# sparsemat/sprs

Measured on NVIDIA H100. Metric: csr_spmv_f64_gflops, higher is better.
Workload: dtype f64

## Files before the change

### include/sprs_b200.h

```cpp
#ifndef SPRS_B200_H
#define SPRS_B200_H

#include <stddef.h>
#include <stdint.h>

#ifdef __cplusplus
extern "C" {
#endif

typedef struct sprs_b200_ctx sprs_b200_ctx;
typedef struct sprs_b200_csmat sprs_b200_csmat;
typedef struct sprs_b200_spgemm sprs_b200_spgemm;

enum { SPRS_B200_CSR = 0, SPRS_B200_CSC = 1 };

enum {
    SPRS_B200_OK = 0,
    SPRS_B200_ERR_DIMENSION = 1,
    SPRS_B200_ERR_STORAGE = 2,
    SPRS_B200_ERR_CUDA = 3,
    SPRS_B200_ERR_NCCL = 4,
    SPRS_B200_ERR_INDEX_RANGE = 5,
    SPRS_B200_ERR_ARGUMENT = 6,
    SPRS_B200_ERR_STRUCTURE = 7,
// ... 186 lines not shown
enum { SPRS_B200_TRI_LOWER = 0, SPRS_B200_TRI_UPPER = 1 };
enum {
    SPRS_B200_SINGULAR_IS_ZERO = 0,
    SPRS_B200_SINGULAR_NUMERIC = 1,
    SPRS_B200_SINGULAR_STRUCTURAL = 2
};
int sprs_b200_trisolve_plan(sprs_b200_ctx* ctx, const sprs_b200_csmat* mat, int tri,
                            sprs_b200_trisolve** out);
int sprs_b200_trisolve_singular(const sprs_b200_trisolve* plan, uint64_t* index, int* reason);
int sprs_b200_trisolve_solve(sprs_b200_trisolve* plan, double* rhs, uint64_t len);
int sprs_b200_trisolve_solve_dev(sprs_b200_trisolve* plan, double* d_rhs, void* stream);
int sprs_b200_trisolve_free(sprs_b200_trisolve* plan);

typedef struct sprs_b200_ldl sprs_b200_ldl;
int sprs_b200_is_symmetric(sprs_b200_ctx* ctx, const sprs_b200_csmat* mat, int* out);
int sprs_b200_diag_solve(sprs_b200_ctx* ctx, const double* diag, double* x, uint64_t len);
int sprs_b200_ldl_symbolic(sprs_b200_ctx* ctx, const sprs_b200_csmat* mat, const uint32_t* perm,
                           int check_symmetry, sprs_b200_ldl** out);
uint64_t sprs_b200_ldl_nnz(const sprs_b200_ldl* ldl);
int sprs_b200_ldl_factor(const sprs_b200_ldl* sym, const sprs_b200_csmat* mat,
                         sprs_b200_ldl** out);
int sprs_b200_ldl_update(sprs_b200_ldl* num, const sprs_b200_csmat* mat);
int sprs_b200_ldl_singular(const sprs_b200_ldl* num, uint64_t* index);
int sprs_b200_ldl_solve(sprs_b200_ldl* num, const double* b, double* x, uint64_t len);
int sprs_b200_ldl_solve_dev(sprs_b200_ldl* num, const double* d_b, double* d_x, void* stream);
int sprs_b200_ldl_get_l(const sprs_b200_ldl* num, uint32_t* colptr, uint32_t* indices,
                        double* data);
int sprs_b200_ldl_get_d(const sprs_b200_ldl* num, double* d, uint64_t len);
int sprs_b200_ldl_free(sprs_b200_ldl* ldl);

int sprs_b200_diag_gather_ceiling(sprs_b200_ctx* ctx, const sprs_b200_csmat* mat,
                                  const double* d_x, int iters, double* ms_per_pass,
                                  uint64_t* nnz_covered);

int sprs_b200_gen_rmat_keys(sprs_b200_ctx* ctx, uint64_t seed, int scale, uint64_t n_rows,
                            uint64_t n_cols, double a, double b, double c, uint64_t first,
                            uint64_t count, uint64_t* d_keys, void* stream);
int sprs_b200_gen_uniform_keys(sprs_b200_ctx* ctx, uint64_t seed, uint64_t n_rows,
                               uint64_t n_cols, uint64_t first, uint64_t count,
                               uint64_t* d_keys, void* stream);
int sprs_b200_gen_normal_from_keys(sprs_b200_ctx* ctx, uint64_t seed, const uint64_t* d_keys,
                                   uint64_t count, double* d_out, void* stream);
int sprs_b200_gen_split_keys(sprs_b200_ctx* ctx, const uint64_t* d_keys, uint64_t count,
                             uint32_t* d_rows, uint32_t* d_cols, void* stream);
int sprs_b200_gen_hash_keys(sprs_b200_ctx* ctx, uint64_t seed, const uint64_t* d_keys,
                            uint64_t count, uint64_t* d_out, void* stream);

#ifdef __cplusplus
}
#endif
#endif
```

### rust/sprs-b200-sys/src/lib.rs

```rust
#![allow(non_camel_case_types)]
use std::os::raw::{c_char, c_double, c_int, c_void};

#[repr(C)] pub struct sprs_b200_ctx { _private: [u8; 0] }
#[repr(C)] pub struct sprs_b200_csmat { _private: [u8; 0] }
#[repr(C)] pub struct sprs_b200_spgemm { _private: [u8; 0] }
#[repr(C)] pub struct sprs_b200_comm { _private: [u8; 0] }
#[repr(C)] pub struct sprs_b200_symm { _private: [u8; 0] }
#[repr(C)] pub struct sprs_b200_bicgstab { _private: [u8; 0] }
#[repr(C)] pub struct sprs_b200_trisolve { _private: [u8; 0] }
#[repr(C)] pub struct sprs_b200_ldl { _private: [u8; 0] }

pub const SPRS_B200_CSR: c_int = 0;
pub const SPRS_B200_CSC: c_int = 1;
pub const SPRS_B200_BINOP_ADD: c_int = 0;
pub const SPRS_B200_BINOP_SUB: c_int = 1;
pub const SPRS_B200_BINOP_MUL: c_int = 2;
pub const SPRS_B200_OK: c_int = 0;
pub const SPRS_B200_ERR_DIMENSION: c_int = 1;
pub const SPRS_B200_ERR_STORAGE: c_int = 2;
pub const SPRS_B200_ERR_CUDA: c_int = 3;
pub const SPRS_B200_ERR_NCCL: c_int = 4;
pub const SPRS_B200_ERR_INDEX_RANGE: c_int = 5;
pub const SPRS_B200_ERR_ARGUMENT: c_int = 6;
pub const SPRS_B200_ERR_STRUCTURE: c_int = 7;
// ... 178 lines not shown
    pub fn sprs_b200_comm_unique_id(id: *mut c_char) -> c_int;
    pub fn sprs_b200_comm_init_rank(
        ctx: *mut sprs_b200_ctx, id: *const c_char, rank: c_int, world: c_int,
        out: *mut *mut sprs_b200_comm) -> c_int;
    pub fn sprs_b200_comm_free(comm: *mut sprs_b200_comm) -> c_int;
    pub fn sprs_b200_comm_rank(comm: *const sprs_b200_comm) -> c_int;
    pub fn sprs_b200_comm_world(comm: *const sprs_b200_comm) -> c_int;
    pub fn sprs_b200_comm_multicast_supported(comm: *const sprs_b200_comm) -> c_int;
    pub fn sprs_b200_comm_allgather_host(
        comm: *mut sprs_b200_comm, mine: *const c_void, bytes: u64, all: *mut c_void) -> c_int;
    pub fn sprs_b200_comm_barrier_host(comm: *mut sprs_b200_comm) -> c_int;
    pub fn sprs_b200_comm_barrier_dev(comm: *mut sprs_b200_comm, stream: *mut c_void) -> c_int;
    pub fn sprs_b200_comm_check(comm: *mut sprs_b200_comm, stream: *mut c_void) -> c_int;
    pub fn sprs_b200_symm_alloc(
        comm: *mut sprs_b200_comm, bytes: u64, want_multicast: c_int,
        out: *mut *mut sprs_b200_symm) -> c_int;
    pub fn sprs_b200_symm_free(buf: *mut sprs_b200_symm) -> c_int;
    pub fn sprs_b200_symm_ptr(buf: *const sprs_b200_symm, rank: c_int) -> *mut c_void;
    pub fn sprs_b200_symm_multicast_ptr(buf: *const sprs_b200_symm) -> *mut c_void;
    pub fn sprs_b200_symm_bytes(buf: *const sprs_b200_symm) -> u64;
    pub fn sprs_b200_partition_rows(
        indptr: *const c_void, indptr_bytes: c_int, rows: u64, nparts: c_int, row_cost: c_double,
        bounds: *mut u64) -> c_int;
    pub fn sprs_b200_spmv_rowpart(
        comm: *mut sprs_b200_comm, mat: *const sprs_b200_csmat, d_x: *const c_double,
        y: *mut sprs_b200_symm, row_offset: u64, exchange: c_int, stream: *mut c_void) -> c_int;
    pub fn sprs_b200_mul_mat_vec_rowpart(
        comm: *mut sprs_b200_comm, mat: *const sprs_b200_csmat, x: *mut sprs_b200_symm,
        x_slice: *const c_double, col_offset: u64, col_count: u64, y_slice: *mut c_double,
        y_len: u64) -> c_int;
    pub fn sprs_b200_diag_gather_ceiling(
        ctx: *mut sprs_b200_ctx, mat: *const sprs_b200_csmat, d_x: *const c_double, iters: c_int,
        ms_per_pass: *mut c_double, nnz_covered: *mut u64) -> c_int;
    pub fn sprs_b200_spmv_chunked_push_dev(
        ctx: *mut sprs_b200_ctx, mat: *const sprs_b200_csmat, d_x: *const c_double,
        row_offset: u64, n_targets: c_int, d_y_bufs: *const *mut c_double, accumulate: c_int,
        n_chunks: c_int, stream: *mut c_void) -> c_int;
    pub fn sprs_b200_spgemm_numeric_dev(
        ctx: *mut sprs_b200_ctx, plan: *mut sprs_b200_spgemm, c: *mut *mut sprs_b200_csmat) -> c_int;
    pub fn sprs_b200_spgemm_nprod(plan: *const sprs_b200_spgemm) -> u64;
    pub fn sprs_b200_bicgstab_new_dev(
        ctx: *mut sprs_b200_ctx, mat: *const sprs_b200_csmat, d_x0: *const c_double,
        d_b: *const c_double, n: u64, out: *mut *mut sprs_b200_bicgstab) -> c_int;
    pub fn sprs_b200_bicgstab_get_dev(
        s: *const sprs_b200_bicgstab, which: c_int, d_out: *mut *const c_double) -> c_int;
    pub fn sprs_b200_gen_rmat_keys(
        ctx: *mut sprs_b200_ctx, seed: u64, scale: c_int, n_rows: u64, n_cols: u64, a: c_double,
        b: c_double, c: c_double, first: u64, count: u64, d_keys: *mut u64, stream: *mut c_void) -> c_int;
    pub fn sprs_b200_gen_uniform_keys(
        ctx: *mut sprs_b200_ctx, seed: u64, n_rows: u64, n_cols: u64, first: u64, count: u64,
        d_keys: *mut u64, stream: *mut c_void) -> c_int;
    pub fn sprs_b200_gen_normal_from_keys(
        ctx: *mut sprs_b200_ctx, seed: u64, d_keys: *const u64, count: u64, d_out: *mut c_double,
        stream: *mut c_void) -> c_int;
    pub fn sprs_b200_gen_split_keys(
        ctx: *mut sprs_b200_ctx, d_keys: *const u64, count: u64, d_rows: *mut u32,
        d_cols: *mut u32, stream: *mut c_void) -> c_int;
    pub fn sprs_b200_gen_hash_keys(
        ctx: *mut sprs_b200_ctx, seed: u64, d_keys: *const u64, count: u64, d_out: *mut u64,
        stream: *mut c_void) -> c_int;
}
```

### sprs_b200/_lib.py

```python
import ctypes as C
import os

_HERE = os.path.dirname(os.path.abspath(__file__))
LIB_PATH = os.path.join(_HERE, "libsprs_b200.so")

OK, ERR_DIMENSION, ERR_STORAGE, ERR_CUDA, ERR_NCCL, ERR_INDEX_RANGE, ERR_ARGUMENT, \
    ERR_STRUCTURE, ERR_UNSUPPORTED = range(9)
CSR, CSC = 0, 1
BINOP_ADD, BINOP_SUB, BINOP_MUL = 0, 1, 2
ERR_SINGULAR = 10
ERR_NOT_SYMMETRIC = 11
TRI_LOWER, TRI_UPPER = 0, 1
SINGULAR_IS_ZERO, SINGULAR_NUMERIC, SINGULAR_STRUCTURAL = 0, 1, 2

_vp, _u64, _i64, _int, _dp = C.c_void_p, C.c_uint64, C.c_int64, C.c_int, C.c_void_p
_dense_sig = [_vp, _vp, _dp, _u64, _u64, _i64, _i64, _dp, _u64, _u64, _i64, _i64]

MATVEC_FN = C.CFUNCTYPE(C.c_int, C.c_void_p, C.c_void_p, C.c_void_p, C.c_void_p)

PROTOTYPES = {
    "sprs_b200_version": (_int, []),
    "sprs_b200_ctx_create": (_int, [_int, C.POINTER(_vp)]),
    "sprs_b200_ctx_destroy": (_int, [_vp]),
    "sprs_b200_last_error": (C.c_char_p, [_vp]),
# ... 68 lines not shown
    "sprs_b200_spgemm_free": (_int, [_vp]),
    "sprs_b200_bicgstab_new": (_int, [_vp, _vp, _dp, _dp, _u64, C.POINTER(_vp)]),
    "sprs_b200_bicgstab_new_dev": (_int, [_vp, _vp, _dp, _dp, _u64, C.POINTER(_vp)]),
    "sprs_b200_bicgstab_new_op": (_int, [_vp, _u64, MATVEC_FN, _vp, _dp, _dp, _int,
                                         C.POINTER(_vp)]),
    "sprs_b200_bicgstab_free": (_int, [_vp]),
    "sprs_b200_bicgstab_step": (_int, [_vp, C.POINTER(C.c_double)]),
    "sprs_b200_bicgstab_soft_restart": (_int, [_vp]),
    "sprs_b200_bicgstab_hard_restart": (_int, [_vp]),
    "sprs_b200_bicgstab_solve": (_int, [_vp, C.c_double, _u64, C.POINTER(_int)]),
    "sprs_b200_bicgstab_set_restart_threshold": (_int, [_vp, C.c_double]),
    "sprs_b200_bicgstab_stats": (_int, [_vp, C.POINTER(_u64), C.POINTER(C.c_double)]),
    "sprs_b200_bicgstab_get": (_int, [_vp, _int, _dp, _u64]),
    "sprs_b200_bicgstab_get_dev": (_int, [_vp, _int, C.POINTER(_vp)]),
    "sprs_b200_trisolve_plan": (_int, [_vp, _vp, _int, C.POINTER(_vp)]),
    "sprs_b200_trisolve_singular": (_int, [_vp, C.POINTER(_u64), C.POINTER(_int)]),
    "sprs_b200_trisolve_solve": (_int, [_vp, _dp, _u64]),
    "sprs_b200_trisolve_solve_dev": (_int, [_vp, _dp, _vp]),
    "sprs_b200_trisolve_free": (_int, [_vp]),
    "sprs_b200_diag_solve": (_int, [_vp, _dp, _dp, _u64]),
    "sprs_b200_is_symmetric": (_int, [_vp, _vp, C.POINTER(_int)]),
    "sprs_b200_ldl_symbolic": (_int, [_vp, _vp, _vp, _int, C.POINTER(_vp)]),
    "sprs_b200_ldl_nnz": (_u64, [_vp]),
    "sprs_b200_ldl_factor": (_int, [_vp, _vp, C.POINTER(_vp)]),
    "sprs_b200_ldl_update": (_int, [_vp, _vp]),
    "sprs_b200_ldl_singular": (_int, [_vp, C.POINTER(_u64)]),
    "sprs_b200_ldl_solve": (_int, [_vp, _dp, _dp, _u64]),
    "sprs_b200_ldl_solve_dev": (_int, [_vp, _dp, _dp, _vp]),
    "sprs_b200_ldl_get_l": (_int, [_vp, _vp, _vp, _dp]),
    "sprs_b200_ldl_get_d": (_int, [_vp, _dp, _u64]),
    "sprs_b200_ldl_free": (_int, [_vp]),
    "sprs_b200_diag_gather_ceiling": (_int, [_vp, _vp, _dp, _int, C.POINTER(C.c_double),
                                             C.POINTER(_u64)]),
    "sprs_b200_gen_rmat_keys": (_int, [_vp, _u64, _int, _u64, _u64, C.c_double, C.c_double,
                                       C.c_double, _u64, _u64, _vp, _vp]),
    "sprs_b200_gen_uniform_keys": (_int, [_vp, _u64, _u64, _u64, _u64, _u64, _vp, _vp]),
    "sprs_b200_gen_normal_from_keys": (_int, [_vp, _u64, _vp, _u64, _vp, _vp]),
    "sprs_b200_gen_split_keys": (_int, [_vp, _vp, _u64, _vp, _vp, _vp]),
    "sprs_b200_gen_hash_keys": (_int, [_vp, _u64, _vp, _u64, _vp, _vp]),
}

_NOT_EMULATED = ("sprs_b200_comm_", "sprs_b200_symm_", "sprs_b200_partition_rows",
                 "sprs_b200_spmv_rowpart", "sprs_b200_mul_mat_vec_rowpart", "sprs_b200_diag_",
                 "sprs_b200_csmat_binop", "sprs_b200_csmat_scale",
                 "sprs_b200_trisolve_",
                 "sprs_b200_ldl_", "sprs_b200_is_symmetric", "sprs_b200_diag_solve")
_lib = None


def load():
    global _lib
    if _lib is not None:
        return _lib
    if not os.path.exists(LIB_PATH):
        raise ImportError(
            "libsprs_b200.so is not built (%s): run `python -c 'import __graft_entry__ as g; "
            "g.build()'` or `make -C sprs_b200/csrc`.  sprs_b200 has no CPU fallback." % LIB_PATH)
    lib = C.CDLL(LIB_PATH)
    emulated = os.path.basename(LIB_PATH).startswith("libsprs_b200_emu")
    for name, (res, args) in PROTOTYPES.items():
        if emulated and name.startswith(_NOT_EMULATED) and not hasattr(lib, name):
            continue
        fn = getattr(lib, name)
        fn.restype = res
        fn.argtypes = args
    _lib = lib
# ... 2 lines not shown
```

### sprs_b200/csrc/api.cu

```cuda

#include <algorithm>
#include <mutex>
#include <vector>

#include <cstdlib>

#include "common.cuh"
#include "ptx.cuh"

namespace {

__global__ void make_policies_kernel(uint64_t* out) {
    out[0] = policy_evict_first();
    out[1] = policy_evict_last();
}

thread_local std::string g_create_error;

template <typename Src, typename Dst>
__global__ void convert_rebase_kernel(const Src* __restrict__ in, Dst* __restrict__ out,
                                      uint64_t n, uint64_t base) {
    const uint64_t i = blockIdx.x * (uint64_t)blockDim.x + threadIdx.x;
    if (i < n) out[i] = (Dst)((uint64_t)in[i] - base);
}
// ... 353 lines not shown
    m->d_indptr = const_cast<uint32_t*>(d_indptr);
    m->d_indices = const_cast<uint32_t*>(d_indices);
    m->d_data = const_cast<double*>(d_data);
    m->owns = false;
    int st = spmv_prepare(ctx, m, ctx->stream);
    if (st == SPRS_B200_OK && cudaStreamSynchronize(ctx->stream) != cudaSuccess) {
        sprs_b200_set_error(ctx, "from_device: partition kernel failed");
        st = SPRS_B200_ERR_CUDA;
    }
    if (st != SPRS_B200_OK) {
        sprs_b200_csmat_free(m);
        return st;
    }
    *out = m;
    return SPRS_B200_OK;
}

int sprs_b200_csmat_free(sprs_b200_csmat* m) {
    if (!m) return SPRS_B200_OK;
    if (m->ctx) cudaSetDevice(m->ctx->device);
    if (m->owns && m->pooled && m->ctx) {
        cudaDeviceSynchronize();
        if (m->d_indptr) cudaFreeAsync(m->d_indptr, m->ctx->stream);
        if (m->d_indices) cudaFreeAsync(m->d_indices, m->ctx->stream);
        if (m->d_data) cudaFreeAsync(m->d_data, m->ctx->stream);
    } else if (m->owns) {
        if (m->d_indptr) cudaFree(m->d_indptr);
        if (m->d_indices) cudaFree(m->d_indices);
        if (m->d_data) cudaFree(m->d_data);
    }
    if (m->d_tile_row) cudaFree(m->d_tile_row);
    if (m->d_tile_k) cudaFree(m->d_tile_k);
    if (m->d_carry) cudaFree(m->d_carry);
    if (m->d_hot_col) cudaFree(m->d_hot_col);
    if (m->d_hot_idx) cudaFree(m->d_hot_idx);
    if (m->csr_cache) sprs_b200_csmat_free(m->csr_cache);
    delete m;
    return SPRS_B200_OK;
}

static int csr_of(sprs_b200_ctx* ctx, const sprs_b200_csmat* m, const sprs_b200_csmat** out) {
    if (m->storage == SPRS_B200_CSR) {
        *out = m;
        return SPRS_B200_OK;
    }
    if (!m->csr_cache) {
        sprs_b200_csmat* t = nullptr;
        SPRS_TRY(sprs_b200_csmat_to_other_storage(ctx, m, &t));
        m->csr_cache = t;
    }
    *out = m->csr_cache;
    return SPRS_B200_OK;
}

int sprs_b200_csmat_storage(const sprs_b200_csmat* m) { return m ? m->storage : -1; }
uint64_t sprs_b200_csmat_rows(const sprs_b200_csmat* m) { return m ? m->rows : 0; }
uint64_t sprs_b200_csmat_cols(const sprs_b200_csmat* m) { return m ? m->cols : 0; }
uint64_t sprs_b200_csmat_nnz(const sprs_b200_csmat* m) { return m ? m->nnz : 0; }

int sprs_b200_csmat_download(sprs_b200_ctx* ctx, const sprs_b200_csmat* m, void* indptr,
                             int indptr_bytes, void* indices, int index_bytes, double* data) {
    if (!ctx || !m || !indptr) return SPRS_B200_ERR_ARGUMENT;
    if ((indptr_bytes != 4 && indptr_bytes != 8) || (index_bytes != 4 && index_bytes != 8))
        SPRS_FAIL(ctx, SPRS_B200_ERR_ARGUMENT, "bad index width");
    if (indptr_bytes == 4 && m->nnz > 0xffffffffull)
        SPRS_FAIL(ctx, SPRS_B200_ERR_INDEX_RANGE, "Index type is not large enough for nnz");
// ... 370 lines not shown
```

### sprs_b200/csrc/common.cuh

```cuda
#pragma once
#include <cuda_runtime.h>

#include <cstdint>
#include <cstdio>
#include <cstring>
#include <string>
#include <vector>

#include "../../include/sprs_b200.h"

constexpr int SPRS_E2E_MAX_CHUNKS = 8;
constexpr int SPRS_E2E_DEFAULT_CHUNKS = 8;

struct sprs_b200_ctx {
    int device = 0;
    int sm_count = 132;
    size_t l2_bytes = 0;
    cudaStream_t stream = nullptr;
    std::string last_error;
    uint64_t launches = 0;
    uint64_t pol_evict_first = 0, pol_evict_last = 0;
    void* h_stage = nullptr;
    size_t h_stage_bytes = 0;
    void* d_scratch[4] = {nullptr, nullptr, nullptr, nullptr};
    size_t d_scratch_bytes[4] = {0, 0, 0, 0};
    cudaStream_t side_stream = nullptr;
    cudaEvent_t ev_fork = nullptr, ev_join = nullptr;
    cudaStream_t copy_stream = nullptr;
    cudaEvent_t ev_chunk[SPRS_E2E_MAX_CHUNKS] = {};
    cudaEvent_t ev_copied = nullptr;
};

struct sprs_b200_csmat {
    sprs_b200_ctx* ctx = nullptr;
    int storage = SPRS_B200_CSR;
    uint64_t rows = 0, cols = 0, nnz = 0;
    uint64_t outer = 0, inner = 0;
    int indptr_bytes = 4;
    void* d_indptr = nullptr;
    uint32_t* d_indices = nullptr;
    double* d_data = nullptr;
    bool owns = true;
    bool pooled = false;
    uint32_t* d_tile_row = nullptr;
    void* d_tile_k = nullptr;
    double* d_carry = nullptr;
    uint64_t n_tiles = 0;
    uint32_t* d_hot_col = nullptr;
    uint32_t* d_hot_idx = nullptr;
    uint32_t n_hot = 0;
    mutable sprs_b200_csmat* csr_cache = nullptr;
    mutable std::vector<uint64_t> e2e_tiles, e2e_rows;
    mutable std::vector<uint64_t> push_tiles, push_rows;
};

#define SPRS_FAIL(ctx, code, ...)                                  \
    do {                                                           \
        char _buf[512];                                            \
        snprintf(_buf, sizeof(_buf), __VA_ARGS__);                 \
        sprs_b200_set_error((ctx), _buf);                          \
        return (code);                                             \
    } while (0)

#define SPRS_CUDA(ctx, expr)                                                              \
    do {                                                                                  \
        cudaError_t _e = (expr);                                                          \
        if (_e != cudaSuccess)                                                            \
            SPRS_FAIL((ctx), SPRS_B200_ERR_CUDA, "%s failed: %s (%s:%d)", #expr,          \
                      cudaGetErrorString(_e), __FILE__, __LINE__);                        \
    } while (0)

#define SPRS_TRY(expr)                      \
    do {                                    \
        int _s = (expr);                    \
        if (_s != SPRS_B200_OK) return _s;  \
    } while (0)

void sprs_b200_set_error(const sprs_b200_ctx* ctx, const char* msg);

// ... 84 lines not shown
```

### sprs_b200/csrc/diag.cu

```cuda
#include "common.cuh"
#include "ptx.cuh"

namespace {

constexpr int DIAG_EPL = 8, DIAG_NWARPS = 8, DIAG_CTAS = 2;

__global__ void __launch_bounds__(DIAG_NWARPS * 32, DIAG_CTAS)
    gather_ceiling_kernel(const uint32_t* __restrict__ idx, const double* __restrict__ val,
                          const double* __restrict__ x, double* __restrict__ out,
                          uint64_t n_tiles) {
    constexpr int WT = DIAG_EPL * 32;
    const int lane = threadIdx.x & 31, warp = threadIdx.x >> 5;
    const uint64_t gw = (uint64_t)blockIdx.x * DIAG_NWARPS + warp;
    const uint64_t GW = (uint64_t)gridDim.x * DIAG_NWARPS;
    const uint64_t pol_s = policy_evict_first(), pol_x = policy_evict_last();
    double acc = 0.0;
    uint32_t cn[DIAG_EPL];
    if (gw < n_tiles) {
#pragma unroll
        for (int i = 0; i < DIAG_EPL; ++i) cn[i] = ldg_stream_u32(idx + gw * WT + lane + 32 * i, pol_s);
    }
    for (uint64_t t = gw; t < n_tiles; t += GW) {
        const uint64_t k0 = t * WT;
        double v[DIAG_EPL], xv[DIAG_EPL];
#pragma unroll
        for (int i = 0; i < DIAG_EPL; ++i) xv[i] = ldg_f64_hint(x + cn[i], pol_x);
#pragma unroll
        for (int i = 0; i < DIAG_EPL; ++i) v[i] = ldg_stream_f64(val + k0 + lane + 32 * i, pol_s);
        if (t + GW < n_tiles) {
#pragma unroll
            for (int i = 0; i < DIAG_EPL; ++i)
                cn[i] = ldg_stream_u32(idx + (t + GW) * WT + lane + 32 * i, pol_s);
        }
#pragma unroll
        for (int i = 0; i < DIAG_EPL; ++i) acc = __dadd_rn(acc, __dmul_rn(v[i], xv[i]));
    }
    out[gw * 32 + lane] = acc;
}

}

extern "C" int sprs_b200_diag_gather_ceiling(sprs_b200_ctx* ctx, const sprs_b200_csmat* mat,
                                             const double* d_x, int iters, double* ms_per_pass,
                                             uint64_t* nnz_covered) {
    if (!ctx || !mat || !d_x || !ms_per_pass || iters < 1) return SPRS_B200_ERR_ARGUMENT;
    if (mat->storage != SPRS_B200_CSR)
        SPRS_FAIL(ctx, SPRS_B200_ERR_STORAGE, "Storage mismatch: diag needs a CSR mirror");
    SPRS_CUDA(ctx, cudaSetDevice(ctx->device));
    constexpr int WT = DIAG_EPL * 32;
    const uint64_t n_tiles = mat->nnz / WT;
    if (nnz_covered) *nnz_covered = n_tiles * WT;
    *ms_per_pass = 0.0;
    if (n_tiles == 0) return SPRS_B200_OK;
    cudaStream_t s = ctx->stream;
    uint64_t grid = (uint64_t)ctx->sm_count * DIAG_CTAS;
    const uint64_t need = (n_tiles + DIAG_NWARPS - 1) / DIAG_NWARPS;
    if (grid > need) grid = need;
    void* d_out = nullptr;
    SPRS_TRY(ctx_scratch(ctx, 3, grid * DIAG_NWARPS * 32 * sizeof(double), &d_out));
    SPRS_CUDA(ctx, cudaFuncSetAttribute(gather_ceiling_kernel,
                                        cudaFuncAttributePreferredSharedMemoryCarveout, 0));
    cudaEvent_t e0, e1;
    SPRS_CUDA(ctx, cudaEventCreate(&e0));
    SPRS_CUDA(ctx, cudaEventCreate(&e1));
    for (int i = 0; i < 2; ++i)
        gather_ceiling_kernel<<<(unsigned)grid, DIAG_NWARPS * 32, 0, s>>>(
            mat->d_indices, mat->d_data, d_x, (double*)d_out, n_tiles);
    cudaEventRecord(e0, s);
    for (int i = 0; i < iters; ++i)
        gather_ceiling_kernel<<<(unsigned)grid, DIAG_NWARPS * 32, 0, s>>>(
            mat->d_indices, mat->d_data, d_x, (double*)d_out, n_tiles);
    cudaEventRecord(e1, s);
    cudaError_t e = cudaEventSynchronize(e1);
    float ms = 0.f;
    if (e == cudaSuccess) e = cudaEventElapsedTime(&ms, e0, e1);
    cudaEventDestroy(e0);
    cudaEventDestroy(e1);
    if (e != cudaSuccess) SPRS_FAIL(ctx, SPRS_B200_ERR_CUDA, "diag: %s", cudaGetErrorString(e));
    ctx->launches += (uint64_t)iters + 2;
    *ms_per_pass = (double)ms / iters;
    return SPRS_B200_OK;
}
```

### sprs_b200/csrc/spmv.cu

```cuda

#include "common.cuh"
#include "ptx.cuh"
#include "scan.cuh"

#include <algorithm>
#include <cstdlib>
#include <type_traits>

namespace {

constexpr int SPMV_STAGE_ROWS = 66;
constexpr uint32_t SPMV_ROW_COST = 16;

template <typename P>
__global__ void tile_cut_kernel(const P* __restrict__ indptr, uint32_t rows, uint64_t nnz,
                                uint64_t n_tiles, uint32_t w, uint32_t row_cost,
                                uint32_t* __restrict__ tile_row, P* __restrict__ tile_k) {
    const uint64_t t = blockIdx.x * (uint64_t)blockDim.x + threadIdx.x;
    if (t > n_tiles) return;
    if (t == n_tiles) {
        tile_row[t] = rows;
        tile_k[t] = (P)nnz;
        return;
    }
// ... 159 lines not shown
                        for (int u = 0; u < U; ++u)
                            c[u] = q + (P)(u * 32) < qe ? ldg_stream_u32(indices + q + (P)(u * 32), pol_stream) : 0u;
#pragma unroll
                        for (int u = 0; u < U; ++u)
                            v[u] = q + (P)(u * 32) < qe ? ldg_stream_f64(data + q + (P)(u * 32), pol_stream) : 0.0;
#pragma unroll
                        for (int u = 0; u < U; ++u)
                            xv[u] = q + (P)(u * 32) < qe ? gather_x<HOT>(x, hot, c[u], polx) : 0.0;
#pragma unroll
                        for (int u = 0; u < U; ++u)
                            if (q + (P)(u * 32) < qe) a2 = __dadd_rn(a2, __dmul_rn(v[u], xv[u]));
                    }
#pragma unroll
                    for (int o = 16; o > 0; o >>= 1) a2 = __dadd_rn(a2, __shfl_xor_sync(FULL, a2, o));
                    if (lane == 0) sink_row<MULTI>(k, (uint64_t)rbase + jj, a2);
                }
            }
        }
        if (r_last - rbase < 31) break;
    }
}

template <typename P, int NWARPS, int MINB, int U, bool MULTI, bool HOT>
__global__ void __launch_bounds__(NWARPS * 32, MINB)
    spmv_rows_kernel(const P* __restrict__ indptr, const uint32_t* __restrict__ indices,
                     const double* __restrict__ data, const uint32_t* __restrict__ tile_row,
                     const P* __restrict__ tile_k, const double* __restrict__ x,
                     const __grid_constant__ SpmvTargets yt,
                     double* __restrict__ carry, uint64_t nnz, uint32_t rows, uint32_t t_begin,
                     uint32_t t_end , int accumulate,
                     uint64_t pol_stream , uint64_t polx ,
                     int stage_rows ,
                     const uint32_t* __restrict__ hot_col ,
                     uint32_t n_hot) {
    const int lane = threadIdx.x & 31, warp = threadIdx.x >> 5;
    extern __shared__ __align__(16) double hot_x[];
    if constexpr (HOT) {
        for (uint32_t q = threadIdx.x; q < n_hot; q += NWARPS * 32)
            hot_x[q] = ldg_f64_hint(x + hot_col[q], polx);
        __syncthreads();
    }
    const uint32_t GW = gridDim.x * NWARPS;
    RowSink sink;
    sink.y = yt.p[0];
    sink.yt = &yt;
    sink.accumulate = accumulate;
    sink.stage = nullptr;
    sink.stage_off = 0;
    double* my_stage = nullptr;
    if constexpr (MULTI) {
        __shared__ __align__(16) double stage_all[NWARPS * SPMV_STAGE_ROWS];
        my_stage = stage_all + warp * SPMV_STAGE_ROWS;
    }
    const uint32_t par = MULTI ? (uint32_t)(((uintptr_t)yt.p[1] >> 3) & 1) : 0u;
    uint32_t t = t_begin + blockIdx.x * NWARPS + warp;
    if (t >= t_end) return;
    uint32_t r0 = tile_row[t], r1 = tile_row[t + 1];
    P k0 = tile_k[t], k1 = tile_k[t + 1];
    P b_first = (uint64_t)r0 + lane <= (r1 < rows ? (uint64_t)r1 + 1 : (uint64_t)r1)
                    ? indptr[(size_t)r0 + lane] : (P)0;
    for (;;) {
        const uint32_t tn = t + GW;
        uint32_t r0n = 0, r1n = 0;
        P k0n = 0, k1n = 0;
        if (tn < t_end) {
            r0n = tile_row[tn];
            r1n = tile_row[tn + 1];
            k0n = tile_k[tn];
            k1n = tile_k[tn + 1];
        }
        sink.carry_slot = carry + t;
        sink.r1 = r1;
        if (MULTI && stage_rows) {
            const uint32_t base = (r0 + par) & ~1u;
            const bool fits = r1 > r0 && (r1 + par - base) <= (uint32_t)SPMV_STAGE_ROWS;
            sink.stage = fits ? my_stage : nullptr;
            sink.stage_off = base - par;
            if (fits) {
                if (lane == 0) bulk_wait_group_read0();
                __syncwarp();
            }
        }
        const uint32_t r_last = r1 < rows ? r1 : r1 - 1;
        const uint64_t cnt = k1 - k0, nr = (uint64_t)(r_last - r0) + 1;
#define SPMV_ROWS(G)                                                                            \
    rows_direct<P, G, U, MULTI, HOT>(sink, indptr, indices, data, x, hot_x, k0, k1, r0, r_last,   \
                                     b_first, pol_stream, polx, lane)
        if (cnt <= 24 * nr)
            SPMV_ROWS(4);
        else if (cnt <= 48 * nr)
            SPMV_ROWS(8);
        else if (cnt <= 96 * nr)
            SPMV_ROWS(16);
        else
            SPMV_ROWS(32);
// ... 2 lines not shown
            fence_proxy_async();
            __syncwarp();
            if (lane == 0) {
                uint32_t lo = r0, hi = r1;
                if ((lo + par) & 1u) {
                    const double v = my_stage[lo - sink.stage_off];
                    for (int q = 1; q < yt.n; ++q) yt.p[q][lo] = v;
                    ++lo;
                }
                if ((hi - lo) & 1u) {
                    --hi;
                    const double v = my_stage[hi - sink.stage_off];
                    for (int q = 1; q < yt.n; ++q) yt.p[q][hi] = v;
                }
                if (hi > lo) {
                    for (int q = 1; q < yt.n; ++q)
                        bulk_s2g(yt.p[q] + lo, my_stage + (lo - sink.stage_off), (hi - lo) * 8u);
                    bulk_commit_group();
                }
            }
            sink.stage = nullptr;
        }
        if (tn >= t_end) break;
        const P b_next = (uint64_t)r0n + lane <= (r1n < rows ? (uint64_t)r1n + 1 : (uint64_t)r1n)
                             ? indptr[(size_t)r0n + lane] : (P)0;
        t = tn;
        r0 = r0n;
        r1 = r1n;
        k0 = k0n;
        k1 = k1n;
        b_first = b_next;
    }
    if (MULTI && stage_rows && lane == 0) bulk_wait_group0();
}

__global__ void spmv_fixup_kernel(const uint32_t* __restrict__ tile_row,
                                  const double* __restrict__ carry, SpmvTargets yt,
                                  uint64_t n_tiles) {
    const uint64_t t = blockIdx.x * (uint64_t)blockDim.x + threadIdx.x;
    if (t + 1 >= n_tiles) return;
    const uint32_t row = tile_row[t + 1];
    if (t > 0 && tile_row[t] == row) return;
    uint64_t lo = t + 1, hi = n_tiles - 1;
    for (uint64_t step = 1; lo + step < hi; step <<= 1) {
        if (tile_row[lo + step + 1] > row) {
            hi = lo + step;
            break;
        }
        lo += step;
    }
    while (lo < hi) {
        const uint64_t mid = lo + (hi - lo) / 2;
        if (tile_row[mid + 1] > row)
            hi = mid;
        else
            lo = mid + 1;
    }
    double sum = carry[t];
#pragma unroll 8
    for (uint64_t u = t + 1; u < lo; ++u) sum = __dadd_rn(sum, carry[u]);
    const double v = __dadd_rn(yt.p[0][row], sum);
#pragma unroll
    for (int q = 0; q < SPMV_MAX_TARGETS; ++q)
        if (q < yt.n) yt.p[q][row] = v;
}

// ... 97 lines not shown
            const int dyn = (int)(spmv_hot().k * sizeof(double));
            const int per_cta = dyn + (multi ? nwarps * SPMV_STAGE_ROWS * 8 : 0) + 1024;
            SPRS_CUDA(ctx, cudaFuncSetAttribute(kern, cudaFuncAttributeMaxDynamicSharedMemorySize, dyn));
            carve = (int)((100ull * ctas * per_cta + 228 * 1024 - 1) / (228 * 1024));
        } else {
            carve = multi ? 15 : 0;
            if (const char* e = getenv("SPRS_B200_SPMV_CARVEOUT")) carve = atoi(e);
        }
        SPRS_CUDA(ctx, cudaFuncSetAttribute(kern, cudaFuncAttributePreferredSharedMemoryCarveout,
                                            carve));
        configured = true;
    }
    int stage_rows = 0;
    if (multi) {
        stage_rows = yt.n > 2 ? SPMV_STAGE_ROWS : 0;
        if (const char* e = getenv("SPRS_B200_SPMV_PEER_STORES")) {
            if (e[0] == 'd') stage_rows = 0;
            if (e[0] == 't') stage_rows = SPMV_STAGE_ROWS;
        }
        for (int q = 2; q < yt.n; ++q)
            if ((((uintptr_t)yt.p[q] ^ (uintptr_t)yt.p[1]) >> 3) & 1) stage_rows = 0;
    }
    uint64_t grid = (uint64_t)ctx->sm_count * ctas;
    const uint64_t need = (t1 - t0 + nwarps - 1) / nwarps;
    if (grid > need) grid = need;
    const size_t smem = hot ? m->n_hot * sizeof(double) : 0;
    kern<<<(unsigned)grid, nwarps * 32, smem, s>>>((const P*)m->d_indptr,
                                                   hot ? m->d_hot_idx : m->d_indices,
                                                   m->d_data, m->d_tile_row, (const P*)m->d_tile_k, d_x, yt,
                                                   m->d_carry,
                                                   m->nnz, (uint32_t)m->rows, (uint32_t)t0,
                                                   (uint32_t)t1, accumulate, ctx->pol_evict_first,
                                                   ctx->pol_evict_last, stage_rows, m->d_hot_col,
                                                   m->n_hot);
    return SPRS_B200_OK;
}

__device__ __forceinline__ void add_aggregated(uint32_t* counts, uint32_t key, unsigned active) {
    const unsigned peers = __match_any_sync(active, key);
    if ((int)(threadIdx.x & 31) == __ffs(peers) - 1) atomicAdd(counts + key, (uint32_t)__popc(peers));
}

__global__ void hot_count_kernel(const uint32_t* __restrict__ indices, uint64_t nnz,
                                 uint32_t* __restrict__ counts) {
    const uint64_t stride = (uint64_t)gridDim.x * blockDim.x;
    for (uint64_t base = blockIdx.x * (uint64_t)blockDim.x + (threadIdx.x & ~31u); base < nnz;
         base += stride) {
        const uint64_t i = base + (threadIdx.x & 31);
        const bool valid = i < nnz;
        const unsigned active = __ballot_sync(0xffffffffu, valid);
        if (valid) add_aggregated(counts, indices[i], active);
    }
}

__global__ void hot_count_hist_kernel(const uint32_t* __restrict__ counts, uint32_t cols,
                                      uint32_t hi, uint32_t* __restrict__ hist) {
    const uint64_t stride = (uint64_t)gridDim.x * blockDim.x;
    for (uint64_t base = blockIdx.x * (uint64_t)blockDim.x + (threadIdx.x & ~31u); base < cols;
         base += stride) {
        const uint64_t i = base + (threadIdx.x & 31);
        const uint32_t c = i < cols ? counts[i] : 0u;
        const bool take = c > 0 && (hi == ~0u || (c >> 16) == hi);
        const unsigned active = __ballot_sync(0xffffffffu, take);
        if (take) add_aggregated(hist, hi == ~0u ? c >> 16 : c & 0xffffu, active);
    }
}

// ... 104 lines not shown
    if (m->n_hot == 0) {
        cudaGetLastError();
        if (hot_col) cudaFree(hot_col);
        if (hot_idx) cudaFree(hot_idx);
    }
    if (counts) cudaFree(counts);
    if (hist) cudaFree(hist);
    if (flag) cudaFree(flag);
    if (slot) cudaFree(slot);
    if (d_hot_nnz) cudaFree(d_hot_nnz);
    return st;
}

int check_spmv_args(sprs_b200_ctx* ctx, const sprs_b200_csmat* m) {
    if (m->storage != SPRS_B200_CSR)
        SPRS_FAIL(ctx, SPRS_B200_ERR_STORAGE, "Storage mismatch: spmv needs a CSR mirror");
    if (!m->d_tile_row) SPRS_FAIL(ctx, SPRS_B200_ERR_ARGUMENT, "csmat has no SpMV partition");
    return SPRS_B200_OK;
}

}

int spmv_tile_nnz() { return spmv_variant().wt; }

int spmv_prepare(sprs_b200_ctx* ctx, sprs_b200_csmat* m, cudaStream_t s, bool hot_set) {
    if (m->storage != SPRS_B200_CSR) return SPRS_B200_OK;
    const uint32_t w = (uint32_t)spmv_tile_nnz();
    const uint32_t row_cost = (uint32_t)spmv_variant().row_cost;
    const uint64_t total = m->nnz + (uint64_t)row_cost * m->rows;
    m->n_tiles = total == 0 ? 1 : (total + w - 1) / w;
    SPRS_CUDA(ctx, cudaMalloc((void**)&m->d_tile_row, (m->n_tiles + 1) * sizeof(uint32_t)));
    SPRS_CUDA(ctx, cudaMalloc((void**)&m->d_tile_k, (m->n_tiles + 1) * (size_t)m->indptr_bytes));
    SPRS_CUDA(ctx, cudaMalloc((void**)&m->d_carry, m->n_tiles * sizeof(double)));
    const uint64_t n = m->n_tiles + 1;
    const unsigned grid = (unsigned)((n + 255) / 256);
    if (m->indptr_bytes == 4)
        tile_cut_kernel<uint32_t><<<grid, 256, 0, s>>>((const uint32_t*)m->d_indptr, (uint32_t)m->rows,
                                                       m->nnz, m->n_tiles, w, row_cost, m->d_tile_row,
                                                       (uint32_t*)m->d_tile_k);
    else
        tile_cut_kernel<uint64_t><<<grid, 256, 0, s>>>((const uint64_t*)m->d_indptr, (uint32_t)m->rows,
                                                       m->nnz, m->n_tiles, w, row_cost, m->d_tile_row,
                                                       (uint64_t*)m->d_tile_k);
    ctx->launches += 1;
    SPRS_CUDA(ctx, cudaGetLastError());
    if (hot_set) SPRS_TRY(spmv_prepare_hot(ctx, m, s));
    return SPRS_B200_OK;
}

int spmv_launch_targets(sprs_b200_ctx* ctx, const sprs_b200_csmat* m, const double* d_x,
                        const SpmvTargets& yt, int accumulate, cudaStream_t s) {
    SPRS_TRY(check_spmv_args(ctx, m));
    if (m->rows == 0) return SPRS_B200_OK;
    if (m->indptr_bytes == 4)
        SPRS_TRY(launch_variant<uint32_t>(ctx, m, d_x, yt, accumulate, 0, m->n_tiles, s));
    else
        SPRS_TRY(launch_variant<uint64_t>(ctx, m, d_x, yt, accumulate, 0, m->n_tiles, s));
    ctx->launches += 1;
    if (m->n_tiles > 1) {
        const unsigned fgrid = (unsigned)((m->n_tiles - 1 + 255) / 256);
        spmv_fixup_kernel<<<fgrid, 256, 0, s>>>(m->d_tile_row, m->d_carry, yt, m->n_tiles);
        ctx->launches += 1;
    }
    SPRS_CUDA(ctx, cudaGetLastError());
    return SPRS_B200_OK;
}
// ... 30 lines not shown
```

Measured before the change: 248.4.

## Add dynamic tile scheduling to hot-set SpMV and a hot gather-ceiling probe

In the hot-set SpMV kernel, the fixed grid-stride tile assignment is replaced by an atomic ticket counter, so each warp claims its next tile on the fly. The last warp to finish resets the counter. This targets load imbalance between warps with a persistent grid. It adds one global atomic per tile and a completion counter, and it relies on a per-matrix scratch counter that concurrent launches would share. A hot-set variant of the diagnostic gather-ceiling timer is also added.

Result: faster. 254.1 (median of 6 runs) (+2.3%).

```diff
diff --git a/include/sprs_b200.h b/include/sprs_b200.h
--- a/include/sprs_b200.h
+++ b/include/sprs_b200.h
@@ -242,6 +242,9 @@
 int sprs_b200_diag_gather_ceiling(sprs_b200_ctx* ctx, const sprs_b200_csmat* mat,
                                   const double* d_x, int iters, double* ms_per_pass,
                                   uint64_t* nnz_covered);
+int sprs_b200_diag_gather_ceiling_hot(sprs_b200_ctx* ctx, const sprs_b200_csmat* mat,
+                                      const double* d_x, int iters, double* ms_per_pass,
+                                      uint64_t* nnz_covered);
 
 int sprs_b200_gen_rmat_keys(sprs_b200_ctx* ctx, uint64_t seed, int scale, uint64_t n_rows,
                             uint64_t n_cols, double a, double b, double c, uint64_t first,
diff --git a/rust/sprs-b200-sys/src/lib.rs b/rust/sprs-b200-sys/src/lib.rs
--- a/rust/sprs-b200-sys/src/lib.rs
+++ b/rust/sprs-b200-sys/src/lib.rs
@@ -234,6 +234,9 @@
     pub fn sprs_b200_diag_gather_ceiling(
         ctx: *mut sprs_b200_ctx, mat: *const sprs_b200_csmat, d_x: *const c_double, iters: c_int,
         ms_per_pass: *mut c_double, nnz_covered: *mut u64) -> c_int;
+    pub fn sprs_b200_diag_gather_ceiling_hot(
+        ctx: *mut sprs_b200_ctx, mat: *const sprs_b200_csmat, d_x: *const c_double, iters: c_int,
+        ms_per_pass: *mut c_double, nnz_covered: *mut u64) -> c_int;
     pub fn sprs_b200_spmv_chunked_push_dev(
         ctx: *mut sprs_b200_ctx, mat: *const sprs_b200_csmat, d_x: *const c_double,
         row_offset: u64, n_targets: c_int, d_y_bufs: *const *mut c_double, accumulate: c_int,
diff --git a/sprs_b200/_lib.py b/sprs_b200/_lib.py
--- a/sprs_b200/_lib.py
+++ b/sprs_b200/_lib.py
@@ -124,6 +124,8 @@
     "sprs_b200_ldl_free": (_int, [_vp]),
     "sprs_b200_diag_gather_ceiling": (_int, [_vp, _vp, _dp, _int, C.POINTER(C.c_double),
                                              C.POINTER(_u64)]),
+    "sprs_b200_diag_gather_ceiling_hot": (_int, [_vp, _vp, _dp, _int, C.POINTER(C.c_double),
+                                                 C.POINTER(_u64)]),
     "sprs_b200_gen_rmat_keys": (_int, [_vp, _u64, _int, _u64, _u64, C.c_double, C.c_double,
                                        C.c_double, _u64, _u64, _vp, _vp]),
     "sprs_b200_gen_uniform_keys": (_int, [_vp, _u64, _u64, _u64, _u64, _u64, _vp, _vp]),
diff --git a/sprs_b200/csrc/api.cu b/sprs_b200/csrc/api.cu
--- a/sprs_b200/csrc/api.cu
+++ b/sprs_b200/csrc/api.cu
@@ -409,6 +409,7 @@
     if (m->d_tile_row) cudaFree(m->d_tile_row);
     if (m->d_tile_k) cudaFree(m->d_tile_k);
     if (m->d_carry) cudaFree(m->d_carry);
+    if (m->d_tile_next) cudaFree(m->d_tile_next);
     if (m->d_hot_col) cudaFree(m->d_hot_col);
     if (m->d_hot_idx) cudaFree(m->d_hot_idx);
     if (m->csr_cache) sprs_b200_csmat_free(m->csr_cache);
diff --git a/sprs_b200/csrc/common.cuh b/sprs_b200/csrc/common.cuh
--- a/sprs_b200/csrc/common.cuh
+++ b/sprs_b200/csrc/common.cuh
@@ -45,6 +45,7 @@
     uint32_t* d_tile_row = nullptr;
     void* d_tile_k = nullptr;
     double* d_carry = nullptr;
+    uint32_t* d_tile_next = nullptr;
     uint64_t n_tiles = 0;
     uint32_t* d_hot_col = nullptr;
     uint32_t* d_hot_idx = nullptr;
diff --git a/sprs_b200/csrc/diag.cu b/sprs_b200/csrc/diag.cu
--- a/sprs_b200/csrc/diag.cu
+++ b/sprs_b200/csrc/diag.cu
@@ -4,16 +4,24 @@
 namespace {
 
 constexpr int DIAG_EPL = 8, DIAG_NWARPS = 8, DIAG_CTAS = 2;
+constexpr int DIAG_HOT_NWARPS = 32, DIAG_HOT_CTAS = 1;
+constexpr uint32_t DIAG_HOT_TAG = 0x80000000u;
 
-__global__ void __launch_bounds__(DIAG_NWARPS * 32, DIAG_CTAS)
+template <int NWARPS, int CTAS, bool HOT>
+__global__ void __launch_bounds__(NWARPS * 32, CTAS)
     gather_ceiling_kernel(const uint32_t* __restrict__ idx, const double* __restrict__ val,
                           const double* __restrict__ x, double* __restrict__ out,
-                          uint64_t n_tiles) {
+                          uint64_t n_tiles, const uint32_t* __restrict__ hot_col, uint32_t n_hot) {
     constexpr int WT = DIAG_EPL * 32;
     const int lane = threadIdx.x & 31, warp = threadIdx.x >> 5;
-    const uint64_t gw = (uint64_t)blockIdx.x * DIAG_NWARPS + warp;
-    const uint64_t GW = (uint64_t)gridDim.x * DIAG_NWARPS;
+    const uint64_t gw = (uint64_t)blockIdx.x * NWARPS + warp;
+    const uint64_t GW = (uint64_t)gridDim.x * NWARPS;
     const uint64_t pol_s = policy_evict_first(), pol_x = policy_evict_last();
+    extern __shared__ __align__(16) double hot_x[];
+    if constexpr (HOT) {
+        for (uint32_t q = threadIdx.x; q < n_hot; q += NWARPS * 32) hot_x[q] = ldg_f64_hint(x + hot_col[q], pol_x);
+        __syncthreads();
+    }
     double acc = 0.0;
     uint32_t cn[DIAG_EPL];
     if (gw < n_tiles) {
@@ -24,7 +32,8 @@
         const uint64_t k0 = t * WT;
         double v[DIAG_EPL], xv[DIAG_EPL];
 #pragma unroll
-        for (int i = 0; i < DIAG_EPL; ++i) xv[i] = ldg_f64_hint(x + cn[i], pol_x);
+        for (int i = 0; i < DIAG_EPL; ++i)
+            xv[i] = HOT && (cn[i] & DIAG_HOT_TAG) ? hot_x[cn[i] & ~DIAG_HOT_TAG] : ldg_f64_hint(x + cn[i], pol_x);
 #pragma unroll
         for (int i = 0; i < DIAG_EPL; ++i) v[i] = ldg_stream_f64(val + k0 + lane + 32 * i, pol_s);
         if (t + GW < n_tiles) {
@@ -38,14 +47,13 @@
     out[gw * 32 + lane] = acc;
 }
 
-}
-
-extern "C" int sprs_b200_diag_gather_ceiling(sprs_b200_ctx* ctx, const sprs_b200_csmat* mat,
-                                             const double* d_x, int iters, double* ms_per_pass,
-                                             uint64_t* nnz_covered) {
+template <int NWARPS, int CTAS, bool HOT>
+int time_ceiling(sprs_b200_ctx* ctx, const sprs_b200_csmat* mat, const double* d_x, int iters,
+                 double* ms_per_pass, uint64_t* nnz_covered) {
     if (!ctx || !mat || !d_x || !ms_per_pass || iters < 1) return SPRS_B200_ERR_ARGUMENT;
     if (mat->storage != SPRS_B200_CSR)
         SPRS_FAIL(ctx, SPRS_B200_ERR_STORAGE, "Storage mismatch: diag needs a CSR mirror");
+    if (HOT && mat->n_hot == 0) SPRS_FAIL(ctx, SPRS_B200_ERR_ARGUMENT, "diag: the mirror has no hot set");
     SPRS_CUDA(ctx, cudaSetDevice(ctx->device));
     constexpr int WT = DIAG_EPL * 32;
     const uint64_t n_tiles = mat->nnz / WT;
@@ -53,23 +61,28 @@
     *ms_per_pass = 0.0;
     if (n_tiles == 0) return SPRS_B200_OK;
     cudaStream_t s = ctx->stream;
-    uint64_t grid = (uint64_t)ctx->sm_count * DIAG_CTAS;
-    const uint64_t need = (n_tiles + DIAG_NWARPS - 1) / DIAG_NWARPS;
+    uint64_t grid = (uint64_t)ctx->sm_count * CTAS;
+    const uint64_t need = (n_tiles + NWARPS - 1) / NWARPS;
     if (grid > need) grid = need;
     void* d_out = nullptr;
-    SPRS_TRY(ctx_scratch(ctx, 3, grid * DIAG_NWARPS * 32 * sizeof(double), &d_out));
-    SPRS_CUDA(ctx, cudaFuncSetAttribute(gather_ceiling_kernel,
-                                        cudaFuncAttributePreferredSharedMemoryCarveout, 0));
+    SPRS_TRY(ctx_scratch(ctx, 3, grid * NWARPS * 32 * sizeof(double), &d_out));
+    auto kern = gather_ceiling_kernel<NWARPS, CTAS, HOT>;
+    const size_t smem = HOT ? mat->n_hot * sizeof(double) : 0;
+    const uint32_t* idx = HOT ? mat->d_hot_idx : mat->d_indices;
+    if (HOT)
+        SPRS_CUDA(ctx, cudaFuncSetAttribute(kern, cudaFuncAttributeMaxDynamicSharedMemorySize, (int)smem));
+    const int carve = HOT ? (int)((100ull * CTAS * (smem + 1024) + 228 * 1024 - 1) / (228 * 1024)) : 0;
+    SPRS_CUDA(ctx, cudaFuncSetAttribute(kern, cudaFuncAttributePreferredSharedMemoryCarveout, carve));
     cudaEvent_t e0, e1;
     SPRS_CUDA(ctx, cudaEventCreate(&e0));
     SPRS_CUDA(ctx, cudaEventCreate(&e1));
     for (int i = 0; i < 2; ++i)
-        gather_ceiling_kernel<<<(unsigned)grid, DIAG_NWARPS * 32, 0, s>>>(
-            mat->d_indices, mat->d_data, d_x, (double*)d_out, n_tiles);
+        kern<<<(unsigned)grid, NWARPS * 32, smem, s>>>(idx, mat->d_data, d_x, (double*)d_out, n_tiles,
+                                                       mat->d_hot_col, mat->n_hot);
     cudaEventRecord(e0, s);
     for (int i = 0; i < iters; ++i)
-        gather_ceiling_kernel<<<(unsigned)grid, DIAG_NWARPS * 32, 0, s>>>(
-            mat->d_indices, mat->d_data, d_x, (double*)d_out, n_tiles);
+        kern<<<(unsigned)grid, NWARPS * 32, smem, s>>>(idx, mat->d_data, d_x, (double*)d_out, n_tiles,
+                                                       mat->d_hot_col, mat->n_hot);
     cudaEventRecord(e1, s);
     cudaError_t e = cudaEventSynchronize(e1);
     float ms = 0.f;
@@ -81,3 +94,18 @@
     *ms_per_pass = (double)ms / iters;
     return SPRS_B200_OK;
 }
+
+}
+
+extern "C" int sprs_b200_diag_gather_ceiling(sprs_b200_ctx* ctx, const sprs_b200_csmat* mat,
+                                             const double* d_x, int iters, double* ms_per_pass,
+                                             uint64_t* nnz_covered) {
+    return time_ceiling<DIAG_NWARPS, DIAG_CTAS, false>(ctx, mat, d_x, iters, ms_per_pass, nnz_covered);
+}
+
+extern "C" int sprs_b200_diag_gather_ceiling_hot(sprs_b200_ctx* ctx, const sprs_b200_csmat* mat,
+                                                 const double* d_x, int iters, double* ms_per_pass,
+                                                 uint64_t* nnz_covered) {
+    return time_ceiling<DIAG_HOT_NWARPS, DIAG_HOT_CTAS, true>(ctx, mat, d_x, iters, ms_per_pass,
+                                                              nnz_covered);
+}
diff --git a/sprs_b200/csrc/spmv.cu b/sprs_b200/csrc/spmv.cu
--- a/sprs_b200/csrc/spmv.cu
+++ b/sprs_b200/csrc/spmv.cu
@@ -215,7 +215,7 @@
                      uint64_t pol_stream , uint64_t polx ,
                      int stage_rows ,
                      const uint32_t* __restrict__ hot_col ,
-                     uint32_t n_hot) {
+                     uint32_t n_hot, uint32_t* __restrict__ tile_next ) {
     const int lane = threadIdx.x & 31, warp = threadIdx.x >> 5;
     extern __shared__ __align__(16) double hot_x[];
     if constexpr (HOT) {
@@ -238,12 +238,20 @@
     const uint32_t par = MULTI ? (uint32_t)(((uintptr_t)yt.p[1] >> 3) & 1) : 0u;
     uint32_t t = t_begin + blockIdx.x * NWARPS + warp;
     if (t >= t_end) return;
+    const uint32_t extra = t_end - t_begin > GW ? t_end - t_begin - GW : 0u;
+    uint32_t ticket = 0;
+    if (HOT && lane == 0) ticket = atomicAdd(tile_next, 1u);
     uint32_t r0 = tile_row[t], r1 = tile_row[t + 1];
     P k0 = tile_k[t], k1 = tile_k[t + 1];
     P b_first = (uint64_t)r0 + lane <= (r1 < rows ? (uint64_t)r1 + 1 : (uint64_t)r1)
                     ? indptr[(size_t)r0 + lane] : (P)0;
     for (;;) {
-        const uint32_t tn = t + GW;
+        uint32_t tn = t + GW;
+        if constexpr (HOT) {
+            const uint32_t q = __shfl_sync(0xffffffffu, ticket, 0);
+            tn = q < extra ? t_begin + GW + q : t_end;
+            if (lane == 0 && tn < t_end) ticket = atomicAdd(tile_next, 1u);
+        }
         uint32_t r0n = 0, r1n = 0;
         P k0n = 0, k1n = 0;
         if (tn < t_end) {
@@ -312,6 +320,15 @@
         b_first = b_next;
     }
     if (MULTI && stage_rows && lane == 0) bulk_wait_group0();
+    if (HOT && lane == 0) {
+        __threadfence();
+        const uint32_t active = t_end - t_begin < GW ? t_end - t_begin : GW;
+        if (atomicAdd(tile_next + 1, 1u) == active - 1) {
+            __threadfence();
+            atomicExch(tile_next, 0u);
+            atomicExch(tile_next + 1, 0u);
+        }
+    }
 }
 
 __global__ void spmv_fixup_kernel(const uint32_t* __restrict__ tile_row,
@@ -475,7 +492,7 @@
                                                    m->nnz, (uint32_t)m->rows, (uint32_t)t0,
                                                    (uint32_t)t1, accumulate, ctx->pol_evict_first,
                                                    ctx->pol_evict_last, stage_rows, m->d_hot_col,
-                                                   m->n_hot);
+                                                   m->n_hot, m->d_tile_next);
     return SPRS_B200_OK;
 }
 
@@ -646,6 +663,8 @@
     SPRS_CUDA(ctx, cudaMalloc((void**)&m->d_tile_row, (m->n_tiles + 1) * sizeof(uint32_t)));
     SPRS_CUDA(ctx, cudaMalloc((void**)&m->d_tile_k, (m->n_tiles + 1) * (size_t)m->indptr_bytes));
     SPRS_CUDA(ctx, cudaMalloc((void**)&m->d_carry, m->n_tiles * sizeof(double)));
+    SPRS_CUDA(ctx, cudaMalloc((void**)&m->d_tile_next, 2 * sizeof(uint32_t)));
+    SPRS_CUDA(ctx, cudaMemsetAsync(m->d_tile_next, 0, 2 * sizeof(uint32_t), s));
     const uint64_t n = m->n_tiles + 1;
     const unsigned grid = (unsigned)((n + 255) / 256);
     if (m->indptr_bytes == 4)
```
